# DavidRother/cooking_zoo

Measured on AMD Instinct MI355X. Metric: env-steps/sec at N parallel envs (1/2/4/8 GPU) + achieved HBM GB/s, higher is better.
Workload: dtype u8/u32 state, f64 obs+reward

## Files before the change

cooking_zoo_amd/csrc/cz_api.hip:

```cpp
#include <hip/hip_runtime.h>
#include <dlfcn.h>
#include <stdarg.h>
#include <stdio.h>
#include <stdlib.h>
#include <string.h>

#include <atomic>
#include <string>
#include <vector>

#include "../../include/cookingzoo.h"
#include "cz_launch.h"
#include "cz_generate.h"

using namespace cz;

constexpr int STAT_CHAINS = 256, STAT_COLS = 13;
__global__ __launch_bounds__(64) void k_stats_chains(const uint32_t *__restrict__ su, const double *__restrict__ sf,
                                                     const uint32_t *__restrict__ state, int RW, int N,
                                                     unsigned long long *__restrict__ part ) {
    const int chain = (int)blockIdx.x * 4 + ((int)threadIdx.x >> 4), col = (int)threadIdx.x & 15;
    const int widx = col == 0 ? (int)SU_STEPS : col == 1 ? (int)SU_EPISODES : col == 2 ? (int)SU_LENSUM : col == 3 ? (int)SU_TRUNC
                   : col == 4 ? (int)SU_TERM : col < 9 ? (int)SU_COMPLETED0 + col - 5 : 0;
    const int fidx = (col >= 9 && col < STAT_COLS) ? (int)SF_SUM0 + col - 9 : (int)SF_SUM0;
// ... 283 lines not shown
    void *comm = nullptr;
    int n_ranks = 1, rank = 0;
    int wt_override = -1;
    bool lean_enabled = true;
    bool lean_cfg_enabled = true;
    int last_step_variant = -1;
    int last_step_lean = -1;
    int last_step_mode = -1;
    bool huge = false;
    int instance = 0;
    unsigned long long *tl_base = nullptr;
    int32_t tl_cap = 0;
    int64_t tl_count = 0;
    bool graphs_enabled = true;
    bool ring_fused = false;
    int64_t n_ring_fused_steps = 0;
    int32_t graph_min_run = 48;
    int32_t ring_prefix = 0;
    int32_t ring_split = -1;
    bool few_queues = false;
    hipStream_t split_stream = nullptr;
    hipEvent_t ev_fork = nullptr, ev_join = nullptr;
    size_t zero_copy_bytes = (size_t)256 << 10;
    cz_stats *d_gather = nullptr;
    std::string err;
};

static thread_local std::string g_err;
static int ready(cz_handle h);
static int set_device(cz_handle h);
static int begin_ranged_call(cz_handle h, int64_t b, int64_t c);
static void mark_ranks(cz_handle h, int32_t first, int32_t count, int ok);
static int flush_updates(cz_handle h, bool force);

static int fail(cz_handle h, const char *fmt, ...) {
    char buf[512];
    va_list ap;
    va_start(ap, fmt);
    vsnprintf(buf, sizeof buf, fmt, ap);
    va_end(ap);
    if (h) h->err = buf; else g_err = buf;
    return 1;
}

#define HIPCHK(h, call)                                                                      \
    do {                                                                                     \
        hipError_t _e = (call);                                                              \
        if (_e != hipSuccess) return fail(h, "%s failed: %s", #call, hipGetErrorString(_e)); \
    } while (0)

extern "C" const char *cz_last_error(cz_handle h) { return h ? h->err.c_str() : g_err.c_str(); }

template <class T>
static int64_t read_counter(cz_handle h, const void *d_counter, const char *who) {
    T n = 0;
    if (hipSetDevice(h->cfg.device_id) != hipSuccess || hipStreamSynchronize(h->stream) != hipSuccess ||
        hipMemcpy(&n, d_counter, sizeof n, hipMemcpyDeviceToHost) != hipSuccess) { fail(h, "%s: copy failed", who); return -1; }
    return (int64_t)n;
}
static int pool_levels(cz_handle h, const uint8_t *level_of, int32_t n_levels, const char *misfit, std::vector<uint8_t> &levels) {
    levels.assign((size_t)h->n_layouts, 0);
    for (int i = 0; i < h->n_layouts; ++i) {
        const int lv = level_of ? level_of[i] : 0;
        if (lv >= n_levels) return fail(h, misfit, i, lv, n_levels);
        levels[(size_t)i] = (uint8_t)lv;
    }
// ... 310 lines not shown
    if (!h) return fail(nullptr, "null handle");
    HIPCHK(h, hipStreamSynchronize(h->stream));
    return 0;
}

static int encode_node(cz_handle h, int recipe, uint32_t j, uint32_t hw, uint32_t children, uint32_t *out) {
    const uint32_t cls = hw & 0xFF, cond = (hw >> 8) & 0xFF, counts = (hw >> 24) & 1;
    uint32_t w = children | (counts << 8);
    if (cls < 16) {
        w |= 0x200u | ((cls <= BLENDER ? cls : 7u) << 10);
    } else if (cls < 32) {
        const bool blender_food = (cls - 16) == CARROT || (cls - 16) == BANANA;
        uint32_t acc;
        if (cond & 0x10u) acc = cond & 0xFu;
        else if (cond == COND_NONE) acc = 0xFu;
        else if (cond == COND_CHOPPED) acc = 0xAu;
        else if (cond == COND_NOT_CHOPPED) acc = 0x5u;
        else if (cond == COND_MASHED) acc = blender_food ? 0xCu : 0u;
        else if (cond == COND_NOT_MASHED) acc = blender_food ? 0x3u : 0u;
        else return fail(h, "cz_load_recipes: recipe %d node %u: unknown condition code %u", recipe, j, cond);
        w |= 0x2000u | ((cls - 16) << 16) | (acc << 24);
    }
    *out = w;
    return 0;
}

extern "C" int cz_load_recipes(cz_handle h, const uint32_t *table, int32_t n, int32_t max_nodes) {
    if (!h || !table || n < 1 || n > 255 || (max_nodes != MAX_NODES && max_nodes != WIDE_NODES)) return fail(h, "cz_load_recipes: bad arguments");
    const bool wide = max_nodes == WIDE_NODES;
    const size_t row_words = wide ? 1 + 2 * WIDE_NODES : 1 + MAX_NODES;
    for (int i = 0; i < n; ++i)
        if (table[(size_t)i * row_words] > (uint32_t)max_nodes) return fail(h, "cz_load_recipes: recipe %d has more than %d nodes", i, max_nodes);
    HIPCHK(h, hipSetDevice(h->cfg.device_id));
    if (h->d_recipes) { HIPCHK(h, hipStreamSynchronize(h->stream)); HIPCHK(h, hipFree(h->d_recipes)); h->d_recipes = nullptr; h->P.recipes = nullptr; }
    size_t bytes = (size_t)n * row_words * 4;
    HIPCHK(h, hipMalloc(&h->d_recipes, bytes));
    std::vector<uint32_t> dev(table, table + (size_t)n * row_words);
    for (int i = 0; i < n; ++i) {
        uint32_t *row = dev.data() + (size_t)i * row_words;
        const uint32_t nn = row[0];
        for (uint32_t j = 0; j < (uint32_t)max_nodes; ++j) {
            if (wide) {
                if (j >= nn) { row[1 + 2 * j] = row[2 + 2 * j] = 0; continue; }
                if (encode_node(h, i, j, row[1 + 2 * j], 0, &row[1 + 2 * j])) return 1;
                row[2 + 2 * j] &= 0xFFFFu;
            } else {
                if (j >= nn) { row[1 + j] = 0; continue; }
                if (encode_node(h, i, j, row[1 + j], (row[1 + j] >> 16) & 0xFF, &row[1 + j])) return 1;
            }
        }
        row[0] = nn & 0xFFu;
    }
    HIPCHK(h, hipMemcpyAsync(h->d_recipes, dev.data(), bytes, hipMemcpyHostToDevice, h->stream));
    HIPCHK(h, hipStreamSynchronize(h->stream));
    h->n_recipes = n;
    h->P.recipes = h->d_recipes;
    h->tables_version++;
    h->n_partner = 0;
    h->n_goal_rows = 0;
    int sensitive = h->P.A > 2;
    for (int i = 0; i < n && !sensitive; ++i) {
        const uint32_t *row = table + (size_t)i * row_words;
        auto node = [&](uint32_t j) { return wide ? row[1 + 2 * j] : row[1 + j]; };
        auto kids = [&](uint32_t j) { return wide ? (row[2 + 2 * j] & 0xFFFFu) : ((row[1 + j] >> 16) & 0xFFu); };
        for (uint32_t j = 0; j < row[0] && !sensitive; ++j) {
            uint32_t cls = node(j) & 0xFF, children = kids(j);
            for (uint32_t c = 0; c < row[0]; ++c) {
                if (!((children >> c) & 1)) continue;
                uint32_t ccls = node(c) & 0xFF;
                bool pw = cls == FLOOR || cls == SWITCH || cls == BLOCK, cw = ccls == FLOOR || ccls == SWITCH || ccls == BLOCK;
                bool pd = cls >= 16 && cls < 32, cd = ccls >= 16 && ccls < 32;
                if ((pw && cd) || (pd && cw)) sensitive = 1;
            }
        }
    }
    h->P.walk_touches = sensitive;
    h->P.wide = wide ? 1 : 0;
    return 0;
}

static int validate_layouts(cz_handle h, const char *who, const uint32_t *init_records, const uint32_t *obs_desc, int32_t n) {
    for (size_t i = 0; i < (size_t)n * h->P.F; ++i) {
        uint32_t off = obs_desc[i] & 0xFFFFu, code4 = obs_desc[i] >> 16;
        uint32_t hw = off >> 1, code = code4 >> 2;
        bool ok = !(off & 1u) && !(code4 & 3u) && (code <= 2 || (code >= 4 && code < 4 + 2 * (uint32_t)h->P.A));
        const uint32_t cell0 = h->huge ? Img<16>::CELL0 : Img<1>::CELL0, ag0 = h->huge ? Img<16>::AG0 : Img<1>::AG0;
        const uint32_t zero = h->huge ? Img<16>::ZERO : Img<1>::ZERO;
        if (hw < cell0) ok = ok && (int)(hw / 6) < h->P.D;
        else if (hw < ag0) ok = ok && (int)((hw - cell0) / 4) < h->P.W * h->P.H;
        else if (hw < zero) ok = ok && (int)((hw - ag0) / 8) < h->P.A && ((hw - ag0) & 7u) < 7u;
        else ok = ok && hw == zero;
        if (!ok) return fail(h, "%s: bad observation descriptor %#x at %zu", who, obs_desc[i], i);
    }
    for (int32_t l = 0; l < n; ++l) {
        const uint32_t *r = init_records + (size_t)l * h->P.RW;
        for (int s2 = 0; s2 < h->P.D; ++s2)
            if (slot_dead_but_tagged(r[h->P.dyn0_off + s2], r[h->P.dyn1_off + s2]))
                return fail(h, "%s: layout %d: slot %d is not alive but carries a container tag", who, l, s2);
    }
    return 0;
}

extern "C" int cz_load_layouts(cz_handle h, const uint32_t *init_records, const uint32_t *obs_desc, int32_t n) {
    if (!h || !init_records || !obs_desc || n < 1 || n > 65535) return fail(h, "cz_load_layouts: bad arguments");
    if (validate_layouts(h, "cz_load_layouts", init_records, obs_desc, n)) return 1;
    HIPCHK(h, hipSetDevice(h->cfg.device_id));
    HIPCHK(h, hipStreamSynchronize(h->stream));
    if (h->copy_stream) HIPCHK(h, hipStreamSynchronize(h->copy_stream));
    if (h->n_layouts > 0 && n < h->n_layouts) {
        unsigned long long misfits = 0;
        HIPCHK(h, hipMemsetAsync(h->d_stats_part, 0, sizeof misfits, h->stream));
        hipLaunchKernelGGL(k_layout_misfits, dim3((unsigned)((h->P.N + 255) / 256)), dim3(256), 0, h->stream, h->d_state, h->P.RW, h->P.N,
                           (uint32_t)n, h->d_stats_part);
        HIPCHK(h, hipGetLastError());
        HIPCHK(h, hipMemcpyAsync(&misfits, h->d_stats_part, sizeof misfits, hipMemcpyDeviceToHost, h->stream));
        HIPCHK(h, hipStreamSynchronize(h->stream));
        if (misfits)
            return fail(h, "cz_load_layouts: %llu resident env record(s) refer to layouts >= %d of the pool being replaced (%d layouts); "
                           "cz_reset / cz_set_state them into the new range first, or load a pool that is not smaller",
                        misfits, n, h->n_layouts);
    }
    if (h->d_lay_block) { HIPCHK(h, hipFree(h->d_lay_block)); h->d_lay_block = nullptr; h->d_lay_init = nullptr; h->P.lay_init = nullptr; }
    if (h->d_lay_desc) { HIPCHK(h, hipFree(h->d_lay_desc)); h->d_lay_desc = nullptr; h->P.lay_desc = nullptr; }
    if (h->rank_stream) HIPCHK(h, hipStreamSynchronize(h->rank_stream));
    if (h->d_lay_rank) { HIPCHK(h, hipFree(h->d_lay_rank)); h->d_lay_rank = nullptr; }
    if (h->h_rank_stage) { HIPCHK(h, hipHostFree(h->h_rank_stage)); h->h_rank_stage = nullptr; }
    if (h->h_lay_stage) { HIPCHK(h, hipHostFree(h->h_lay_stage)); h->h_lay_stage = nullptr; }
    size_t b0 = (size_t)n * h->P.RW * 4, b1 = (size_t)n * h->P.F * 4;
    HIPCHK(h, hipMalloc(&h->d_lay_block, LAY_CTL_WORDS * 4 + b0));
    h->d_lay_init = h->d_lay_block + LAY_CTL_WORDS;
    HIPCHK(h, hipMalloc(&h->d_lay_desc, b1 + 16));
    HIPCHK(h, hipMemsetAsync(h->d_lay_block, 0, LAY_CTL_WORDS * 4, h->stream));
    HIPCHK(h, hipMemsetD32Async((hipDeviceptr_t)(h->d_lay_block + LC_GROUPS), 1, 1, h->stream));
    HIPCHK(h, hipMemsetAsync(h->d_lay_desc, 0, b1 + 16, h->stream));
    const size_t b2 = (size_t)n * h->P.W * h->P.H * sizeof(uint16_t);
    HIPCHK(h, hipMalloc(&h->d_lay_rank, b2));
    HIPCHK(h, hipMemsetAsync(h->d_lay_rank, 0, b2, h->stream));
    h->rank_ok.assign((size_t)n, 0);
    h->rank_missing = n;
    HIPCHK(h, hipMemcpyAsync(h->d_lay_init, init_records, b0, hipMemcpyHostToDevice, h->stream));
    HIPCHK(h, hipMemcpyAsync(h->d_lay_desc, obs_desc, b1, hipMemcpyHostToDevice, h->stream));
    HIPCHK(h, hipStreamSynchronize(h->stream));
    h->n_layouts = n;
    if (h->P.auto_reset & 2) h->spawn_layouts = -1;
    h->lay_groups = 1; h->lay_active = 0; h->upd_ranges.clear(); h->staged_on_copy.clear(); h->staged_on_main.clear(); h->copy_pending = false;
    h->tables_version++;
    h->P.lay_init = h->d_lay_init; h->P.lay_desc = h->d_lay_desc; h->P.L = n;
    return 0;
}

static int flush_updates(cz_handle h, bool force) {
    if (h->upd_ranges.empty()) return 0;
    const hipError_t q = hipEventQuery(h->ev_steps_issued);
    if (q != hipSuccess) (void)hipGetLastError();
    if (q != hipSuccess && !force) return 0;
    const hipStream_t st = q == hipSuccess ? h->copy_stream : h->stream;
    const size_t RWb = (size_t)h->P.RW * 4, Fb = (size_t)h->P.F * 4, L = (size_t)h->n_layouts;
    for (const auto &r : h->upd_ranges) {
        HIPCHK(h, hipMemcpyAsync(h->d_lay_init + (size_t)r.first * h->P.RW, h->h_lay_stage + (size_t)r.first * RWb, (size_t)r.count * RWb,
                                 hipMemcpyHostToDevice, st));
        HIPCHK(h, hipMemcpyAsync(h->d_lay_desc + (size_t)r.first * h->P.F, h->h_lay_stage + L * RWb + (size_t)r.first * Fb, (size_t)r.count * Fb,
                                 hipMemcpyHostToDevice, st));
    }
    if (st == h->copy_stream) {
        if (!h->staged_on_copy.empty() && hipEventQuery(h->ev_copy_done) == hipSuccess) h->staged_on_copy.clear();
        (void)hipGetLastError();
        HIPCHK(h, hipEventRecord(h->ev_copy_done, h->copy_stream));
        h->copy_pending = true;
        h->staged_on_copy.insert(h->staged_on_copy.end(), h->upd_ranges.begin(), h->upd_ranges.end());
    } else {
        if (!h->staged_on_main.empty() && hipEventQuery(h->ev_main_copy_done) == hipSuccess) h->staged_on_main.clear();
        (void)hipGetLastError();
        HIPCHK(h, hipEventRecord(h->ev_main_copy_done, h->stream));
        h->staged_on_main.insert(h->staged_on_main.end(), h->upd_ranges.begin(), h->upd_ranges.end());
    }
    h->upd_ranges.clear();
    return 0;
}

extern "C" int cz_update_layouts(cz_handle h, int32_t first, int32_t count, const uint32_t *init_records, const uint32_t *obs_desc) {
    if (ready(h)) return 1;
    if (first < 0 || count < 0 || first + count > h->n_layouts || (count > 0 && (!init_records || !obs_desc)))
        return fail(h, "cz_update_layouts: slots [%d, %d) outside the resident pool of %d layouts", first, first + count, h ? h->n_layouts : 0);
    if (count > 0 && validate_layouts(h, "cz_update_layouts", init_records, obs_desc, count)) return 1;
    if (set_device(h)) return 1;
    if (caller_capturing(h)) return fail(h, "cz_update_layouts: not inside a stream capture of the caller (it records an event on the captured stream)");
    const size_t RWb = (size_t)h->P.RW * 4, Fb = (size_t)h->P.F * 4, L = (size_t)h->n_layouts;
    if (!h->copy_stream) {
        HIPCHK(h, hipStreamCreateWithFlags(&h->copy_stream, hipStreamNonBlocking));
        HIPCHK(h, hipEventCreateWithFlags(&h->ev_copy_done, hipEventDisableTiming));
        HIPCHK(h, hipEventCreateWithFlags(&h->ev_steps_issued, hipEventDisableTiming));
        HIPCHK(h, hipEventCreateWithFlags(&h->ev_main_copy_done, hipEventDisableTiming));
    }
    if (!h->h_lay_stage) HIPCHK(h, hipHostMalloc((void **)&h->h_lay_stage, L * (RWb + Fb), hipHostMallocDefault));
    if (count == 0) return 0;
// ... 122 lines not shown
    G.img_ag0 = h->huge ? Img<16>::AG0 : Img<1>::AG0; G.img_zero = h->huge ? Img<16>::ZERO : Img<1>::ZERO;
    h->gen_layouts = h->n_layouts;
    return 0;
}

extern "C" int cz_generate_layouts(cz_handle h, int32_t first, int32_t count, uint64_t seed, uint32_t generation) {
    if (ready(h)) return 1;
    if (!h->d_gen_tables || h->gen_layouts != h->n_layouts)
        return fail(h, "cz_generate_layouts: level programs not loaded for this pool (cz_load_level_programs, again after cz_load_layouts)");
    if (first < 0 || count < 0 || (int64_t)first + count > h->n_layouts)
        return fail(h, "cz_generate_layouts: slots [%d, %d) outside the resident pool of %d layouts", first, first + count, h->n_layouts);
    if (count == 0) return 0;
    if (h->lay_groups > 1)
        for (int s = first; s < first + count; ++s) {
            const auto &sl = h->gen_slices[(size_t)s];
            const int part = sl.count / h->lay_groups;
            if (part > 0 && (s - sl.first) / part == h->lay_active)
                return fail(h, "cz_generate_layouts: slot %d is in part %d of its pool slice, which the envs draw from (cz_set_layout_group)", s, h->lay_active);
        }
    if (set_device(h)) return 1;
    if (caller_capturing(h)) {
        if (!h->upd_ranges.empty() || h->copy_pending)
            return fail(h, "cz_generate_layouts: a cz_update_layouts copy is outstanding, which a stream capture cannot be ordered behind");
    } else {
        if (flush_updates(h, true)) return 1;
        if (h->copy_pending) { HIPCHK(h, hipStreamWaitEvent(h->stream, h->ev_copy_done, 0)); h->copy_pending = false; }
    }
    if (h->P.RW > (CELL_WORD0 + 256 + 2 * 255 + 15) / 16 * 16) return fail(h, "cz_generate_layouts: record longer than the generator's staging");
    GenParams G = h->gen;
    G.lay_init = h->d_lay_init; G.lay_desc = h->d_lay_desc; G.lay_rank = h->d_lay_rank;
    G.seed = seed; G.generation = generation; G.first = first;
    hipLaunchKernelGGL(k_generate_layouts, dim3((unsigned)count), dim3(64), 0, h->stream, G);
    HIPCHK(h, hipGetLastError());
    h->n_layout_updates += count;
    mark_ranks(h, first, count, 1);
    return 0;
}
extern "C" int64_t cz_generate_failures(cz_handle h) {
    if (!h) return -1;
    if (!h->d_gen_tables) return 0;
    return read_counter<uint32_t>(h, h->d_gen_tables, "cz_generate_failures");
}

static int copy_back_and_wait(cz_handle h, hipError_t rc, void *dst, const void *src, size_t bytes) {
    if (rc == hipSuccess && dst) rc = hipMemcpyAsync(dst, src, bytes, hipMemcpyDeviceToHost, h->stream);
    const hipError_t rs = hipStreamSynchronize(h->stream);
    HIPCHK(h, rc);
    HIPCHK(h, rs);
    return 0;
}

static void mark_ranks(cz_handle h, int32_t first, int32_t count, int ok) {
    for (int32_t l = first; l < first + count; ++l) {
        h->rank_missing += (int)h->rank_ok[(size_t)l] - ok;
        h->rank_ok[(size_t)l] = (uint8_t)ok;
    }
}
static int check_range(cz_handle h, int64_t b, int64_t c) {
    if (!h) return fail(nullptr, "null handle");
    if (b < 0 || c < 0 || b + c > h->P.N) return fail(h, "env range [%lld, %lld) outside [0, %d)", (long long)b, (long long)(b + c), h->P.N);
    return 0;
}

extern "C" int cz_set_state(cz_handle h, int64_t b, int64_t c, const uint32_t *records) {
    if (check_range(h, b, c)) return 1;
    if (c == 0) return 0;
// ... 1249 lines not shown
```

cooking_zoo_amd/csrc/cz_device.h:

```cpp
#pragma once
#include <hip/hip_runtime.h>
#include <stdint.h>
#include <type_traits>

namespace cz {

constexpr int MAX_AGENTS = 4;
constexpr int MAX_NODES = 8;
constexpr int WIDE_NODES = 16;
constexpr int HDR_WORDS = 8;
constexpr int AGENT_WORD0 = HDR_WORDS;
constexpr int RET_WORD0 = HDR_WORDS + MAX_AGENTS;
constexpr int CELL_WORD0 = RET_WORD0 + 2 * MAX_AGENTS;

enum : uint32_t { FLOOR = 0, COUNTER, DELIVERSQUARE, SWITCH, BLOCK, CUTBOARD, BLENDER };
enum : uint32_t { PLATE = 0, ONION, TOMATO, LETTUCE, CARROT, CUCUMBER, BANANA, APPLE, WATERMELON, BREAD };
enum : uint32_t { CELL_TYPE = 7, CELL_READY = 8, CELL_TOGGLE = 16, CELL_ACTIVE = 32, CELL_WALK = 64 };
enum : uint32_t { D_ALIVE = 1u << 24, D_CHOPPED = 2u << 24, D_MASHED = 4u << 24, D_FREE = 8u << 24, D_DONE = 6u << 24 };
enum : uint32_t { COND_NONE = 0, COND_CHOPPED, COND_MASHED, COND_NOT_CHOPPED, COND_NOT_MASHED };
enum : uint32_t { W_T = 0, W_MARKS, W_LAYOUT, W_STATUS, W_EPISODE, W_RECIPES, W_POOL, W_MARKS_HI };
enum : uint32_t { ST_DONE = 1, ST_TERM = 2, ST_TRUNC = 4 };
constexpr int LUT_Y0 = 63, LUT_ZERO = 126, LUT_ONE = 127;
constexpr int LUT_NDONE0 = 128, LUT_CH0 = 132, LUT_MA0 = 136, LUT_CF0 = 140, LUT_OR0 = 144;
enum : uint32_t { SU_EPISODES = 0, SU_STEPS, SU_LENSUM, SU_TRUNC, SU_TERM, SU_COMPLETED0, SU_LAST_LENGTH = 9, SU_LAST_EPISODE, SU_LAST_FLAGS,
// ... 95 lines not shown
#define CZ_PRIO 1
#endif
#if CZ_PRIO
#define CZ_SETPRIO(p) __builtin_amdgcn_s_setprio(p)
#else
#define CZ_SETPRIO(p) do { } while (0)
#endif
__device__ __forceinline__ uint32_t rfl(uint32_t v) { return __builtin_amdgcn_readfirstlane(v); }
__device__ __forceinline__ uint32_t rdl(uint32_t v, int l) { return __builtin_amdgcn_readlane(v, l); }
__device__ __forceinline__ uint64_t ballot(bool p) { return __builtin_amdgcn_ballot_w64(p); }
__device__ __forceinline__ bool lanes(uint64_t m) { return __builtin_amdgcn_inverse_ballot_w64(m); }
extern "C" __device__ uint32_t __cz_writelane(uint32_t, uint32_t, uint32_t) __asm("llvm.amdgcn.writelane.i32");
__device__ __forceinline__ uint32_t wrl(uint32_t value, int lane, uint32_t into) { return __cz_writelane(value, (uint32_t)lane, into); }

__host__ __device__ inline uint32_t action_hash(uint64_t seed, int64_t env_global, int agent, uint32_t step, uint32_t n) {
    uint32_t x = (uint32_t)seed ^ ((uint32_t)(seed >> 32) * 0x9E3779B1u);
    x ^= (uint32_t)env_global * 0x85EBCA6Bu + (uint32_t)((uint64_t)env_global >> 32) * 0x27D4EB2Fu;
    x ^= ((uint32_t)agent + 1u) * 0xC2B2AE35u;
    x ^= (step + 1u) * 0x165667B1u;
    x ^= x >> 16; x *= 0x7FEB352Du; x ^= x >> 15; x *= 0x846CA68Bu; x ^= x >> 16;
    x += step * 0x9E3779B9u;
    x ^= x >> 16; x *= 0x7FEB352Du; x ^= x >> 15; x *= 0x846CA68Bu; x ^= x >> 16;
    return (uint32_t)(((uint64_t)x * (uint64_t)n) >> 32);
}
__host__ __device__ inline uint32_t next_layout(int64_t env_global, uint32_t episode, uint32_t pool_word, uint32_t n_layouts,
                                                uint32_t groups = 1u, uint32_t active = 0u) {
    uint32_t base = pool_word & 0xFFFFu, count = pool_word >> 16;
    if (count == 0) { base = 0; count = n_layouts; }
    if (groups > 1u) { count /= groups; base += active * count; }
    return base + (uint32_t)(((uint64_t)env_global + (uint64_t)episode * 7919u) % count);
}
constexpr int LAY_CTL_WORDS = 16;
enum : uint32_t { LC_GROUPS = 0, LC_ACTIVE = 1 };

struct SpawnCfg {
    uint64_t seed;
    double despawn_rate, respawn_rate;
    uint32_t grace_period;
    uint32_t stride;
    const uint8_t *areas;
    const uint8_t *level_of_layout;
    uint32_t *exhausted;
};
static_assert(sizeof(SpawnCfg) == 56, "layout of the block behind Params::lut");
constexpr uint32_t SPAWN_CFG_OFFSET = 256 * 8 + 64 * 4;
constexpr uint32_t COORD_TABLE_OFFSET = SPAWN_CFG_OFFSET + 56, ROWSEL_TABLE_OFFSET = COORD_TABLE_OFFSET + 1024 * 4;
constexpr uint32_t LUT_BLOCK_BYTES = ROWSEL_TABLE_OFFSET + 64 * 4;
constexpr int SPAWN_GONE0 = 8, SPAWN_GRACE0 = 12;
__host__ __device__ inline uint32_t spawn_grace_bits(uint32_t grace_period, int n_agents) { return grace_period <= 31u ? 5u : 20u / (uint32_t)n_agents; }
__host__ __device__ inline uint32_t spawn_max_grace(int n_agents) { const uint32_t b = 20u / (uint32_t)n_agents; return b > 5u ? (1u << b) - 1u : 31u; }
__host__ __device__ inline uint32_t spawn_initial_status(uint32_t packed_grace, int n_agents) {
    const uint32_t grace = packed_grace & 0xFFFFFFu, bits = packed_grace >> 24;
    uint32_t st = 0;
    for (int a = 0; a < n_agents; ++a) st |= grace << (SPAWN_GRACE0 + bits * a);
    return st;
}

enum : uint32_t { HDR_LAYOUT = 1u, HDR_RECIPE = 2u, HDR_POOL = 4u };
__host__ __device__ inline uint32_t record_header_faults(uint32_t layout, uint32_t recipes, uint32_t pool, uint32_t L, int R, uint32_t n_recipes) {
    uint32_t faults = layout < L ? 0u : HDR_LAYOUT;
    for (int k = 0; k < R; ++k)
        if (((recipes >> (8 * k)) & 0xFFu) >= n_recipes) faults |= HDR_RECIPE;
    const uint32_t base = pool & 0xFFFFu, count = pool >> 16;
    if (count && base + count > L) faults |= HDR_POOL;
    return faults;
}
// ... 813 lines not shown
```

cooking_zoo_amd/csrc/cz_kernels.h:

```cpp
#pragma once
#include "cz_device.h"
#include <type_traits>

namespace cz {

#ifdef CZ_PROFILE
#define CZ_STAMP(i)                                                                                    \
    do {                                                                                               \
        unsigned long long _t;                                                                         \
        __builtin_amdgcn_sched_barrier(0);                                                             \
        asm volatile("s_memrealtime %0\n\ts_waitcnt lgkmcnt(0)" : "=s"(_t)::"memory");                 \
        __builtin_amdgcn_sched_barrier(0);                                                             \
        if (lane == 0 && P.stamps) P.stamps[(size_t)env * 16 + (i)] = _t;                               \
    } while (0)
#elif defined(CZ_MARKERS)
#define CZ_STAMP(i) asm volatile("; CZ_MARK " #i)
#else
#define CZ_STAMP(i) do { } while (0)
#endif

typedef const __attribute__((address_space(4))) Params *KParams;
struct StepArgsMirror { uint32_t *a; const int32_t *b; const double *c; int32_t i[8]; Params p; };
struct LeanArgsMirror { uint32_t *a; const int32_t *b; const double *c; int32_t i[8]; LeanParams p; };
static_assert(offsetof(LeanArgsMirror, p) == LEADING_SCALAR_BYTES && offsetof(StepArgsMirror, p) == LEADING_SCALAR_BYTES, "leading scalars");
// ... 153 lines not shown

template <class PB>
__device__ __forceinline__ uint32_t load_row_selector(const PB &P, int lane) { return ldg<uint32_t>(P.lut, ROWSEL_TABLE_OFFSET + (uint32_t)lane * 4u); }
template <class PB>
__device__ __forceinline__ uint32_t load_recipe_rows(const PB &P, uint32_t recipes, uint32_t sel) {
    const uint32_t id = (recipes >> (sel & 0xFFu)) & 0xFFu;
    return ldg<uint32_t>(P.recipes, __umul24(id, (1u + MAX_NODES) * 4u) + (sel >> 8));
}
template <class PB>
__device__ __forceinline__ uint32_t load_recipe_rows(const PB &P, uint32_t recipes, int lane) {
    return load_recipe_rows(P, recipes, load_row_selector(P, lane));
}

template <int OPL, int CPL, int NA, bool LEAN = false, class PB>
__device__ __forceinline__ void all_marks(const PB &P, Env<OPL, CPL, NA> &e, const Ctx &cx, uint32_t rowv, Lds<CPL> &s) {
    uint32_t lo = 0, hi = 0;
    if (!LEAN && __builtin_expect(P.wide != 0, 0)) {
#pragma nounroll
        for (int r = 0; r < P.R; ++r) {
            const uint32_t id = (e.recipes >> (8 * r)) & 0xFFu;
            const uint32_t m = Ops<OPL, CPL, NA, 3>::recipe_marks_wide(e, cx, P.recipes + (size_t)id * (1 + 2 * WIDE_NODES), s.locs);
            if (r < 2) lo |= m << (16 * r); else hi |= m << (16 * (r - 2));
        }
    } else {
        if constexpr (CPL <= 4) {
            lo = Ops<OPL, CPL, NA, 3>::recipe_marks_cells(e, cx, rowv, 0xFu, P.R, s.locs);
        } else {
#pragma nounroll
            for (int r = 0; r < P.R; ++r) lo |= Ops<OPL, CPL, NA, 3>::recipe_marks(e, cx, rowv, 9 * r, s.locs) << (8 * r);
        }
    }
    e.marks = lo; e.marks_hi = hi;
}

template <class PB>
__device__ __forceinline__ uint32_t load_submask(const PB &P, int lane) { return ldg<uint32_t>(P.lut, (uint32_t)(LUT_SIZE * 8 + lane * 4)); }

__device__ __forceinline__ void init_lut(const Params &P, double *lut, int tid, int nthreads) {
    for (int i = tid; i < LUT_SIZE; i += nthreads) lut[i] = ldg<double>(P.lut, (uint32_t)i * 8u);
}

template <int CPL> struct CoordWords { uint32_t w[CPL]; };
template <int CPL, class PB>
__device__ __forceinline__ CoordWords<CPL> load_coord_words(const PB &P, int lane) {
    CoordWords<CPL> cw;
#pragma unroll
    for (int k = 0; k < CPL; ++k) cw.w[k] = ldg<uint32_t>(P.lut, COORD_TABLE_OFFSET + (uint32_t)(lane + 64 * k) * 4u);
    return cw;
}
template <int CPL>
__device__ __forceinline__ void init_lds(const Ctx &cx, Lds<CPL> &s, const CoordWords<CPL> &cw) {
    const int lane = cx.lane;
    s.img[Img<CPL>::ZERO] = (uint16_t)(LUT_ABSENT * 8);
    uint32_t *img32 = reinterpret_cast<uint32_t *>(s.img);
#pragma unroll
    for (int k = 0; k < CPL; ++k) {
        const uint32_t c = (uint32_t)(lane + 64 * k);
        img32[(Img<CPL>::CELL0 >> 1) + 2 * c] = cw.w[k];
    }
}
template <int CPL, class PB>
__device__ __forceinline__ void init_lds(const PB &P, const Ctx &cx, Lds<CPL> &s) {
    const int lane = cx.lane;
    s.img[Img<CPL>::ZERO] = (uint16_t)(LUT_ABSENT * 8);
    uint32_t *img32 = reinterpret_cast<uint32_t *>(s.img);
#pragma unroll
// ... 186 lines not shown
        else { CZ_OBS_WRITE_ROWS(0); }
#undef CZ_OBS_WRITE_ROWS
    }
    if (!LEAN && P.F > 128 * OBS_PAIRS) load_desc(P, e.layout, 0, cx.lane, dsc);
    __builtin_amdgcn_wave_barrier();
}

struct StepOut {
    double myrew;
    uint32_t term, trunc;
    bool stepped, finished;
    bool header;
    uint32_t gone;
#ifdef CZ_TIMELINE
    uint32_t dbg;
#endif
};

#define CZ_RARE(hint, x) ((hint) ? __builtin_expect(!!(x), 0) : !!(x))
template <int OPL, int CPL, int NA, int SCHEME, bool FUSED, bool LEAN, class PB>
__device__ __forceinline__ void step_env(const PB &P, unsigned kp_off, Env<OPL, CPL, NA> &e, const Ctx &cx, uint32_t acts,
                                         int64_t env_global, uint32_t &rowv, Lds<CPL> &lds, uint32_t (&dsc)[OBS_CHUNK], Dirty &dt, StepOut &o) {
    using O = Ops<OPL, CPL, NA, SCHEME>;
    o.myrew = 0.0;
    o.term = 0; o.trunc = 0; o.stepped = false; o.finished = false; o.header = false; o.gone = 0u;
#ifdef CZ_TIMELINE
    o.dbg = 0u;
#endif
    const bool spawning = !LEAN && (P.auto_reset & 2) != 0;
    const SpawnCfg *const spawn_cfg = reinterpret_cast<const SpawnCfg *>(reinterpret_cast<const char *>(P.lut) + SPAWN_CFG_OFFSET);
    if (CZ_RARE(FUSED, (e.status & ST_DONE) != 0u)) {
        o.header = true;
        if (P.auto_reset & 1) {
            e.episode += 1;
            const uint32_t *const lay0 = late_params<block_of<PB>>(kp_off)->lay_init;
            typedef const __attribute__((address_space(4))) uint32_t *kconst_u32;
            const kconst_u32 ctl = (kconst_u32)(lay0 - LAY_CTL_WORDS);
            uint32_t lay = next_layout(env_global, e.episode, e.pool, (uint32_t)P.L, ctl[LC_GROUPS], ctl[LC_ACTIVE]);
            uint32_t recipes = e.recipes, episode = e.episode, pool = e.pool;
            load_env<OPL, CPL, NA, LEAN>(P, e, cx, lay0 + (size_t)lay * P.RW);
            e.t = 0; e.layout = lay; e.status = 0; e.episode = episode; e.recipes = recipes; e.pool = pool;
            if (spawning) {
                typedef const __attribute__((address_space(4))) SpawnCfg *kcfg;
                e.status = spawn_initial_status(((kcfg)spawn_cfg)->grace_period, NA);
            }
            all_marks<OPL, CPL, NA, LEAN>(P, e, cx, rowv, lds);
            if (LEAN || P.obs) load_desc(P, lay, 0, cx.lane, dsc);
            dt.cells = 1; dt.touched = 1; dt.interacted = 1;
        } else {
            o.term = (e.status & ST_TERM) ? 1u : 0u;
            o.trunc = (e.status & ST_TRUNC) ? 1u : 0u;
        }
        return;
    }
    o.stepped = true;
    e.t += 1;
#if defined(CZ_PROFILE)
    const int lane = cx.lane; const long long env = env_global - P.env_id_base;
#endif
    O::perform_agent_actions(e, cx, acts, dt);
    CZ_STAMP(2);
    O::progress_and_link(e, cx, dt);
    if (spawning) {
        o.gone = O::handle_agent_spawn(e, cx, spawn_cfg, env_global);
        o.header = true;
    }
    CZ_STAMP(3);
    const bool truncated = (int)e.t >= P.max_steps;
    const uint32_t before = e.marks;
    uint32_t after = before;
    o.myrew = cx.lane < NA ? P.reward_idle : 0.0;
    if (dt.moved & (uint32_t)P.walk_touches) { dt.touched = 1; dt.kinds = ~0ull; }
    if (dt.kinds & 0xFull) dt.kinds = ~0ull;
    bool done = false;
    if (!LEAN && __builtin_expect(P.wide != 0, 0)) {
        if (dt.touched) {
            uint32_t lo = 0, hi = 0;
#pragma nounroll
            for (int r = 0; r < P.R; ++r) {
                const uint32_t id = (e.recipes >> (8 * r)) & 0xFFu;
// ... 398 lines not shown
```

cooking_zoo_amd/csrc/cz_launch.h:

```cpp
#pragma once
#include "cz_kernels.h"
#include "cz_offstep.h"
#include "cz_query.h"

namespace cz {

struct Launchers {
    hipError_t (*step)(const Params &, hipStream_t, StepChoice);
    hipError_t (*reset)(const Params &, hipStream_t, int64_t, int, const int32_t *, const uint32_t *, const uint32_t *, double *);
    hipError_t (*observe)(const Params &, hipStream_t, int64_t, int, double *, uint8_t *);
    bool has_lean;
    hipError_t (*observe_f32)(const Params &, hipStream_t, int64_t, int, float *);
    hipError_t (*reset_where)(const Params &, hipStream_t, const uint8_t *, const int32_t *, double *, float *, uint8_t *, unsigned long long *);
    hipError_t (*restore_where)(const Params &, hipStream_t, const int32_t *, const uint32_t *, int64_t, uint32_t, double *, float *, uint8_t *,
                                unsigned long long *);
    hipError_t (*set_tasks)(const Params &, hipStream_t, const uint8_t *, const uint32_t *, const uint32_t *, uint32_t, uint64_t, uint32_t,
                            unsigned long long *);
    hipError_t (*observe_grid)(const Params &, hipStream_t, int64_t, int, int32_t, uint32_t *, uint8_t *, float *, int32_t *);
    hipError_t (*navigate)(const Params &, hipStream_t, int64_t, int, int32_t, uint32_t, const int32_t *, int32_t *, int32_t *, uint16_t *);
    hipError_t (*partner)(const Params &, hipStream_t, int, const PartnerArgs &);
    hipError_t (*action_effects)(const Params &, hipStream_t, int, const EffectsArgs &);
    hipError_t (*render)(const Params &, hipStream_t, int, const RenderArgs &);
};

template <int OPL, int CPL, bool HAS_LEAN = false>
struct Inst {
    static hipError_t step(const Params &P, hipStream_t st, StepChoice c) {
        if constexpr (HAS_LEAN) {
            if (c.lean && c.cfg >= 0) {
                if (c.cfg != lean_cfg_of(P)) return hipErrorInvalidValue;
                const LeanParams B = lean_block_of(P);
                int row = 0;
#define CZ_X(a, s, r, ea, wt) if (c.cfg == row++) return launch_step_kernel<CPL>(k_step_lean_cfg<OPL, CPL, a, s, r, ea, wt>, P, B, st);
                CZ_LEAN_CFGS(CZ_X)
#undef CZ_X
                return hipErrorInvalidValue;
            }
        }
        return with_agents(P.A, [&](auto na) {
            return with_scheme(P.scheme, [&](auto scheme) {
                constexpr int NA = decltype(na)::value, S = decltype(scheme)::value;
                if (c.lean) {
                    if constexpr (HAS_LEAN) return launch_step_kernel<CPL>(k_step_lean<OPL, CPL, NA, S>, P, lean_block_of(P), st);
                    return hipErrorInvalidValue;
                }
                switch (c.mode) {
                case STEP: return launch_step_kernel<CPL>(k_step<OPL, CPL, NA, S, STEP>, P, st);
                case ROLLOUT: return launch_step_kernel<CPL>(k_step<OPL, CPL, NA, S, ROLLOUT>, P, st);
                case ROLLOUT_ACTIONS: return launch_step_kernel<CPL>(k_step<OPL, CPL, NA, S, ROLLOUT_ACTIONS>, P, st);
                case STEP_CODES: return launch_step_kernel<CPL>(k_step<OPL, CPL, NA, S, STEP_CODES>, P, st);
// ... 4 lines not shown
                case ROLLOUT_ACTIONS_F32: return launch_step_kernel<CPL>(k_step<OPL, CPL, NA, S, ROLLOUT_ACTIONS_F32>, P, st);
                }
                return hipErrorInvalidValue;
            });
        });
    }
#define CZ_LAUNCH_PER_ENV(K, envs, ...)                                                                                             \
    with_agents(P.A, [&](auto na) {                                                                                                 \
        hipLaunchKernelGGL((K<OPL, CPL, decltype(na)::value>), dim3((unsigned)(envs)), dim3(64), 0, st, P, __VA_ARGS__);            \
        return hipGetLastError();                                                                                                   \
    })
    static hipError_t reset(const Params &P, hipStream_t st, int64_t b, int n, const int32_t *lay, const uint32_t *rec,
                            const uint32_t *pool, double *obs) {
        return CZ_LAUNCH_PER_ENV(k_reset, n, b, lay, rec, pool, obs);
    }
    static hipError_t observe(const Params &P, hipStream_t st, int64_t b, int n, double *obs, uint8_t *codes) {
        return CZ_LAUNCH_PER_ENV(k_observe, n, b, obs, codes);
    }
    static hipError_t observe_f32(const Params &P, hipStream_t st, int64_t b, int n, float *obs) {
        return CZ_LAUNCH_PER_ENV(k_observe_f32, n, b, obs);
    }
    static hipError_t reset_where(const Params &P, hipStream_t st, const uint8_t *mask, const int32_t *lay, double *obs, float *obs32,
                                  uint8_t *codes, unsigned long long *refused) {
        return CZ_LAUNCH_PER_ENV(k_reset_where, P.N, mask, lay, obs, obs32, codes, refused);
    }
    static hipError_t restore_where(const Params &P, hipStream_t st, const int32_t *slot, const uint32_t *records, int64_t capacity,
                                    uint32_t n_recipes, double *obs, float *obs32, uint8_t *codes, unsigned long long *refused) {
        return CZ_LAUNCH_PER_ENV(k_restore_where, P.N, slot, records, capacity, n_recipes, obs, obs32, codes, refused);
    }
    static hipError_t set_tasks(const Params &P, hipStream_t st, const uint8_t *mask, const uint32_t *ids, const uint32_t *list, uint32_t K,
                                uint64_t seed, uint32_t n_recipes, unsigned long long *refused) {
        return CZ_LAUNCH_PER_ENV(k_set_tasks, P.N, mask, ids, list, K, seed, n_recipes, refused);
    }
    static hipError_t observe_grid(const Params &P, hipStream_t st, int64_t b, int n, int32_t extended, uint32_t *bits, uint8_t *grid8,
                                   float *grid32, int32_t *agent_xy) {
        return CZ_LAUNCH_PER_ENV(k_observe_grid, n, b, extended, bits, grid8, grid32, agent_xy);
    }
    static hipError_t navigate(const Params &P, hipStream_t st, int64_t b, int n, int32_t T, uint32_t flags, const int32_t *target,
                               int32_t *action, int32_t *steps, uint16_t *field) {
        return CZ_LAUNCH_PER_ENV(k_navigate, n, b, T, flags, target, action, steps, field);
    }
    static hipError_t partner(const Params &P, hipStream_t st, int n, const PartnerArgs &G) { return CZ_LAUNCH_PER_ENV(k_partner, n, G); }
    static hipError_t action_effects(const Params &P, hipStream_t st, int n, const EffectsArgs &G) {
        return with_agents(P.A, [&](auto na) {
            return with_scheme(P.scheme, [&](auto scheme) {
                constexpr int NA = decltype(na)::value, S = decltype(scheme)::value;
                hipLaunchKernelGGL((k_action_effects<OPL, CPL, NA, S>), dim3((unsigned)n * (unsigned)NA), dim3(64), 0, st, P, G);
                return hipGetLastError();
            });
        });
    }
    static hipError_t render(const Params &P, hipStream_t st, int n, const RenderArgs &G) {
        return with_agents(P.A, [&](auto na) {
            hipLaunchKernelGGL((k_render<OPL, CPL, decltype(na)::value>), dim3((unsigned)n * (unsigned)P.H, (G.P + RENDER_BAND - 1u) / RENDER_BAND), dim3(RENDER_THREADS), 0, st,
                               P, G);
            return hipGetLastError();
        });
    }
#undef CZ_LAUNCH_PER_ENV
    static Launchers launchers() {
        Launchers L{};
        L.step = &step; L.reset = &reset; L.observe = &observe; L.has_lean = HAS_LEAN; L.observe_f32 = &observe_f32;
        L.reset_where = &reset_where; L.restore_where = &restore_where; L.observe_grid = &observe_grid; L.navigate = &navigate;
        L.partner = &partner; L.action_effects = &action_effects; L.render = &render; L.set_tasks = &set_tasks;
        return L;
    }
};

Launchers launchers_small();
Launchers launchers_large();
Launchers launchers_huge();

}
```

cooking_zoo_amd/csrc/cz_offstep.h:

```cpp
#pragma once
#include "cz_kernels.h"

namespace cz {

__device__ __forceinline__ void init_lut_f32(const Params &P, float *lutf, int lane) {
    for (int i = lane; i < LUT_SIZE; i += 64) lutf[i] = (float)ldg<double>(P.lut, (uint32_t)i * 8u);
}
template <class T>
__device__ __forceinline__ T *row_of(T *base, size_t i, size_t pitch) { return base ? base + i * pitch : nullptr; }
template <int OPL, int CPL, int NA>
__device__ __forceinline__ void write_forms(const Params &P, const Env<OPL, CPL, NA> &e, const Ctx &cx, Lds<CPL> &lds, double *lut, float *lutf,
                                            double *obs, float *obs32, uint8_t *codes, size_t row) {
    const uint32_t submask = load_submask(P, cx.lane);
    if (obs || codes) {
        if (obs) init_lut(P, lut, cx.lane, 64);
        uint32_t dsc[OBS_CHUNK];
        load_desc(P, e.layout, 0, cx.lane, dsc);
        observe(P, e, cx, lds, lut, dsc, submask, row_of(obs, row, (size_t)NA * P.F), true, true, row_of(codes, row, (size_t)NA * codes_pitch(P.F)));
    }
    if (obs32) {
        init_lut_f32(P, lutf, cx.lane);
        if (!(obs || codes)) build_image<OPL, CPL, NA>(P, e, cx, lds, submask, true, true);
        write_rows_f32<OPL, CPL, NA>(P, e, cx, lds, lutf, obs32 + row * NA * P.F, nullptr);
    }
}
template <int OPL, int CPL, int NA>
__device__ __forceinline__ void begin_episode(const Params &P, Env<OPL, CPL, NA> &e, const Ctx &cx, Lds<CPL> &lds, uint32_t *rec, uint32_t lay,
                                              uint32_t episode, uint32_t recipes, uint32_t pool) {
    load_env(P, e, cx, P.lay_init + (size_t)lay * P.RW);
    e.t = 0; e.layout = lay; e.status = 0; e.episode = episode; e.recipes = recipes; e.pool = pool;
    if (P.auto_reset & 2)
        e.status = spawn_initial_status(rfl(reinterpret_cast<const SpawnCfg *>(reinterpret_cast<const char *>(P.lut) + SPAWN_CFG_OFFSET)->grace_period), NA);
    uint32_t rowv = load_recipe_rows(P, e.recipes, cx.lane);
    all_marks(P, e, cx, rowv, lds);
    store_env(P, e, cx, rec, true, true);
    if (cx.lane < MAX_AGENTS) reinterpret_cast<double *>(rec + RET_WORD0)[cx.lane] = 0.0;
}

template <int OPL, int CPL, int NA>
__global__ __launch_bounds__(64) void k_reset(const Params P, int64_t env_begin, const int32_t *__restrict__ layout_ids,
                                              const uint32_t *__restrict__ recipe_words, const uint32_t *__restrict__ pool_words,
                                              double *obs_out) {
    __shared__ Lds<CPL> lds;
    __shared__ double lut[LUT_SIZE];
    const int i = blockIdx.x;
    Ctx cx{P.W, P.H, P.D, P.W * P.H, (int)threadIdx.x};
    init_lds<CPL>(P, cx, lds);
    Env<OPL, CPL, NA> e;
    uint32_t *rec = P.state + (size_t)(env_begin + i) * P.RW;
    const uint32_t old_episode = rfl(rec[W_EPISODE]);
    begin_episode(P, e, cx, lds, rec, rfl((uint32_t)layout_ids[i]), old_episode, rfl(recipe_words[i]), rfl(pool_words[i]));
    write_forms(P, e, cx, lds, lut, nullptr, obs_out, nullptr, nullptr, (size_t)i);
}

template <int OPL, int CPL, int NA>
__global__ __launch_bounds__(64) void k_observe(const Params P, int64_t env_begin, double *obs_out, uint8_t *codes_out) {
    __shared__ Lds<CPL> lds;
    __shared__ double lut[LUT_SIZE];
    const int i = blockIdx.x;
    Ctx cx{P.W, P.H, P.D, P.W * P.H, (int)threadIdx.x};
    init_lds<CPL>(P, cx, lds);
    Env<OPL, CPL, NA> e;
    load_env(P, e, cx, P.state + (size_t)(env_begin + i) * P.RW);
    write_forms(P, e, cx, lds, lut, nullptr, obs_out, nullptr, codes_out, (size_t)i);
}

template <int OPL, int CPL, int NA>
__global__ __launch_bounds__(64) void k_observe_f32(const Params P, int64_t env_begin, float *obs_out) {
    __shared__ Lds<CPL> lds;
    __shared__ float lutf[LUT_SIZE];
    const int i = blockIdx.x;
    Ctx cx{P.W, P.H, P.D, P.W * P.H, (int)threadIdx.x};
    init_lds<CPL>(P, cx, lds);
    Env<OPL, CPL, NA> e;
    load_env(P, e, cx, P.state + (size_t)(env_begin + i) * P.RW);
    write_forms(P, e, cx, lds, nullptr, lutf, nullptr, obs_out, nullptr, (size_t)i);
}

template <int OPL, int CPL, int NA>
__global__ __launch_bounds__(64) void k_reset_where(const Params P, const uint8_t *__restrict__ mask, const int32_t *__restrict__ layout_ids,
                                                    double *obs_out, float *obs32_out, uint8_t *codes_out, unsigned long long *refused) {
    __shared__ Lds<CPL> lds;
    __shared__ double lut[LUT_SIZE];
    __shared__ float lutf[LUT_SIZE];
    const uint32_t env = blockIdx.x;
    const int lane = (int)threadIdx.x;
    uint32_t *rec = P.state + (size_t)env * P.RW;
    uint32_t old_status = 0u;
    if (mask) {
        if (rfl((uint32_t)mask[env]) == 0u) return;
        old_status = rfl(rec[W_STATUS]);
    } else {
        old_status = rfl(rec[W_STATUS]);
        if (!(old_status & ST_DONE)) return;
    }
    const int32_t want = layout_ids ? (int32_t)rfl((uint32_t)layout_ids[env]) : -1;
    if (want >= P.L) {
        if (lane == 0) atomicAdd(refused, 1ull);
        return;
    }
    const uint32_t old_t = rfl(rec[W_T]), episode = rfl(rec[W_EPISODE]) + 1u, recipes = rfl(rec[W_RECIPES]), pool = rfl(rec[W_POOL]);
    if (!(old_status & ST_DONE) && lane == 0) P.stat_u[(size_t)env * SU_WORDS + SU_STEPS] += old_t;
    uint32_t lay = (uint32_t)want;
    if (want < 0) {
        const uint32_t *ctl = P.lay_init - LAY_CTL_WORDS;
        lay = next_layout(P.env_id_base + (int64_t)env, episode, pool, (uint32_t)P.L, rfl(ctl[LC_GROUPS]), rfl(ctl[LC_ACTIVE]));
    }
    Ctx cx{P.W, P.H, P.D, P.W * P.H, lane};
    init_lds<CPL>(P, cx, lds);
    Env<OPL, CPL, NA> e;
    begin_episode(P, e, cx, lds, rec, lay, episode, recipes, pool);
    write_forms(P, e, cx, lds, lut, lutf, obs_out, obs32_out, codes_out, env);
}

template <int OPL, int CPL>
constexpr int record_chunks() { return ((CELL_WORD0 + 16 * CPL + 128 * OPL + 15) / 16 * 16 + 63) / 64; }
template <int OPL, int CPL, int NA>
__global__ __launch_bounds__(64) void k_restore_where(const Params P, const int32_t *__restrict__ slot, const uint32_t *__restrict__ records,
                                                      int64_t capacity, uint32_t n_recipes, double *obs_out, float *obs32_out,
                                                      uint8_t *codes_out, unsigned long long *refused) {
    __shared__ Lds<CPL> lds;
    __shared__ double lut[LUT_SIZE];
    __shared__ float lutf[LUT_SIZE];
    constexpr int NW = record_chunks<OPL, CPL>();
    const uint32_t env = blockIdx.x;
    const int lane = (int)threadIdx.x;
    int64_t s = (int64_t)env;
    if (slot) {
        const int32_t v = (int32_t)rfl((uint32_t)slot[env]);
        if (v < 0) return;
        s = v;
    }
    if (s >= capacity) {
        if (lane == 0) atomicAdd(refused, 1ull);
        return;
    }
    const uint32_t *row = records + (size_t)s * P.RW;
    uint32_t *rec = P.state + (size_t)env * P.RW;
    const uint32_t RW = (uint32_t)P.RW;
    uint32_t raw[NW];
#pragma unroll
    for (int k = 0; k < NW; ++k) raw[k] = ldg<uint32_t>(row, min((uint32_t)lane + 64u * k, RW - 1u) * 4u);
    Ctx cx{P.W, P.H, P.D, P.W * P.H, lane};
    Env<OPL, CPL, NA> e;
// ... 32 lines not shown
    const int lane = (int)threadIdx.x;
    uint32_t *rec = P.state + (size_t)env * P.RW;
    if (mask) {
        if (rfl((uint32_t)mask[env]) == 0u) return;
    } else {
        if (rfl(rec[W_T]) != 0u) return;
    }
    uint32_t want;
    if (ids) want = rfl(ids[env]);
    else want = rfl(list[task_draw(seed, P.env_id_base + (int64_t)env, rfl(rec[W_EPISODE]), K)]);
    bool bad = false;
    for (int r = 0; r < MAX_AGENTS; ++r) {
        if (r >= P.R) want |= 0xFFu << (8 * r);
        else if (((want >> (8 * r)) & 0xFFu) >= n_recipes) bad = true;
    }
    if (bad) {
        if (lane == 0) atomicAdd(refused, 1ull);
        return;
    }
    Ctx cx{P.W, P.H, P.D, P.W * P.H, lane};
    Env<OPL, CPL, NA> e;
    load_env(P, e, cx, rec);
    e.recipes = want;
    const uint32_t rowv = load_recipe_rows(P, e.recipes, lane);
    all_marks(P, e, cx, rowv, lds);
    uint32_t h = 0;
    h = wrl(e.marks, W_MARKS, h);
    h = wrl(e.recipes, W_RECIPES, h);
    h = wrl(e.marks_hi, W_MARKS_HI, h);
    const uint32_t ul = (uint32_t)lane;
    if (ul == W_MARKS || ul == W_RECIPES || (P.wide && ul == W_MARKS_HI)) stg<uint32_t>(rec, ul * 4u, h);
}

}
```

Before: 779.7 million.

## Precompute per-layout recipe marks table and use it on episode reset

Adds a per-layout table of initial recipe marks, indexed by layout and recipe id and stored after the layout init records. A new kernel fills it whenever layouts or recipes change. On auto-reset and begin_episode, the marks are then read with one small load per lane instead of rerunning all_marks over the recipe rows. This takes the recipe-evaluation work out of the hot reset path, at the cost of extra memory and upkeep every time layouts or recipes are updated.

```diff
diff --git a/cooking_zoo_amd/csrc/cz_api.hip b/cooking_zoo_amd/csrc/cz_api.hip
--- a/cooking_zoo_amd/csrc/cz_api.hip
+++ b/cooking_zoo_amd/csrc/cz_api.hip
@@ -339,6 +339,7 @@
 static int begin_ranged_call(cz_handle h, int64_t b, int64_t c);
 static void mark_ranks(cz_handle h, int32_t first, int32_t count, int ok);
 static int flush_updates(cz_handle h, bool force);
+static int refresh_layout_marks(cz_handle h, int32_t first, int32_t count, hipStream_t st);
 
 static int fail(cz_handle h, const char *fmt, ...) {
     char buf[512];
@@ -715,7 +716,11 @@
     for (int i = 0; i < n; ++i)
         if (table[(size_t)i * row_words] > (uint32_t)max_nodes) return fail(h, "cz_load_recipes: recipe %d has more than %d nodes", i, max_nodes);
     HIPCHK(h, hipSetDevice(h->cfg.device_id));
-    if (h->d_recipes) { HIPCHK(h, hipStreamSynchronize(h->stream)); HIPCHK(h, hipFree(h->d_recipes)); h->d_recipes = nullptr; h->P.recipes = nullptr; }
+    if (h->d_recipes) {
+        HIPCHK(h, hipStreamSynchronize(h->stream));
+        if (h->copy_stream) HIPCHK(h, hipStreamSynchronize(h->copy_stream));
+        HIPCHK(h, hipFree(h->d_recipes)); h->d_recipes = nullptr; h->P.recipes = nullptr;
+    }
     size_t bytes = (size_t)n * row_words * 4;
     HIPCHK(h, hipMalloc(&h->d_recipes, bytes));
     std::vector<uint32_t> dev(table, table + (size_t)n * row_words);
@@ -759,6 +764,17 @@
     }
     h->P.walk_touches = sensitive;
     h->P.wide = wide ? 1 : 0;
+    if (h->P.lay_init) {
+        if (h->copy_stream) HIPCHK(h, hipStreamSynchronize(h->copy_stream));
+        HIPCHK(h, hipMemsetAsync(const_cast<uint16_t *>(lay_marks_of(h->d_lay_init, h->n_layouts, h->P.RW)), 0, lay_marks_bytes(h->n_layouts), h->stream));
+        if (refresh_layout_marks(h, 0, h->n_layouts, h->stream)) return 1;
+    }
+    return 0;
+}
+
+static int refresh_layout_marks(cz_handle h, int32_t first, int32_t count, hipStream_t st) {
+    if (!h->P.recipes || !h->P.lay_init || count <= 0) return 0;
+    HIPCHK(h, h->kl.layout_marks(h->P, st, first, count, (uint32_t)h->n_recipes));
     return 0;
 }
 
@@ -810,11 +826,12 @@
     if (h->h_rank_stage) { HIPCHK(h, hipHostFree(h->h_rank_stage)); h->h_rank_stage = nullptr; }
     if (h->h_lay_stage) { HIPCHK(h, hipHostFree(h->h_lay_stage)); h->h_lay_stage = nullptr; }
     size_t b0 = (size_t)n * h->P.RW * 4, b1 = (size_t)n * h->P.F * 4;
-    HIPCHK(h, hipMalloc(&h->d_lay_block, LAY_CTL_WORDS * 4 + b0));
+    HIPCHK(h, hipMalloc(&h->d_lay_block, LAY_CTL_WORDS * 4 + b0 + lay_marks_bytes(n)));
     h->d_lay_init = h->d_lay_block + LAY_CTL_WORDS;
     HIPCHK(h, hipMalloc(&h->d_lay_desc, b1 + 16));
     HIPCHK(h, hipMemsetAsync(h->d_lay_block, 0, LAY_CTL_WORDS * 4, h->stream));
     HIPCHK(h, hipMemsetD32Async((hipDeviceptr_t)(h->d_lay_block + LC_GROUPS), 1, 1, h->stream));
+    HIPCHK(h, hipMemsetAsync(const_cast<uint16_t *>(lay_marks_of(h->d_lay_init, n, h->P.RW)), 0, lay_marks_bytes(n), h->stream));
     HIPCHK(h, hipMemsetAsync(h->d_lay_desc, 0, b1 + 16, h->stream));
     const size_t b2 = (size_t)n * h->P.W * h->P.H * sizeof(uint16_t);
     HIPCHK(h, hipMalloc(&h->d_lay_rank, b2));
@@ -829,7 +846,7 @@
     h->lay_groups = 1; h->lay_active = 0; h->upd_ranges.clear(); h->staged_on_copy.clear(); h->staged_on_main.clear(); h->copy_pending = false;
     h->tables_version++;
     h->P.lay_init = h->d_lay_init; h->P.lay_desc = h->d_lay_desc; h->P.L = n;
-    return 0;
+    return refresh_layout_marks(h, 0, n, h->stream);
 }
 
 static int flush_updates(cz_handle h, bool force) {
@@ -844,6 +861,7 @@
                                  hipMemcpyHostToDevice, st));
         HIPCHK(h, hipMemcpyAsync(h->d_lay_desc + (size_t)r.first * h->P.F, h->h_lay_stage + L * RWb + (size_t)r.first * Fb, (size_t)r.count * Fb,
                                  hipMemcpyHostToDevice, st));
+        if (refresh_layout_marks(h, r.first, r.count, st)) return 1;
     }
     if (st == h->copy_stream) {
         if (!h->staged_on_copy.empty() && hipEventQuery(h->ev_copy_done) == hipSuccess) h->staged_on_copy.clear();
@@ -1032,6 +1050,7 @@
     G.seed = seed; G.generation = generation; G.first = first;
     hipLaunchKernelGGL(k_generate_layouts, dim3((unsigned)count), dim3(64), 0, h->stream, G);
     HIPCHK(h, hipGetLastError());
+    if (refresh_layout_marks(h, first, count, h->stream)) return 1;
     h->n_layout_updates += count;
     mark_ranks(h, first, count, 1);
     return 0;
diff --git a/cooking_zoo_amd/csrc/cz_device.h b/cooking_zoo_amd/csrc/cz_device.h
--- a/cooking_zoo_amd/csrc/cz_device.h
+++ b/cooking_zoo_amd/csrc/cz_device.h
@@ -151,6 +151,11 @@
 }
 constexpr int LAY_CTL_WORDS = 16;
 enum : uint32_t { LC_GROUPS = 0, LC_ACTIVE = 1 };
+constexpr int LAY_MARK_IDS = 256;
+constexpr size_t lay_marks_bytes(int L) { return (size_t)L * LAY_MARK_IDS * sizeof(uint16_t); }
+__host__ __device__ inline const uint16_t *lay_marks_of(const uint32_t *lay_init, int L, int RW) {
+    return reinterpret_cast<const uint16_t *>(lay_init + (size_t)L * (size_t)RW);
+}
 
 struct SpawnCfg {
     uint64_t seed;
diff --git a/cooking_zoo_amd/csrc/cz_kernels.h b/cooking_zoo_amd/csrc/cz_kernels.h
--- a/cooking_zoo_amd/csrc/cz_kernels.h
+++ b/cooking_zoo_amd/csrc/cz_kernels.h
@@ -209,6 +209,25 @@
     }
     e.marks = lo; e.marks_hi = hi;
 }
+template <class PB>
+__device__ __forceinline__ uint32_t load_fresh_marks(const PB &P, const uint32_t *lay0, uint32_t lay, uint32_t recipes, int lane) {
+    const uint32_t id = (recipes >> (8u * ((uint32_t)lane & 3u))) & 0xFFu;
+    return ldg<uint16_t>(lay_marks_of(lay0, P.L, P.RW), (lay * (uint32_t)LAY_MARK_IDS + id) * 2u);
+}
+template <int OPL, int CPL, int NA, bool LEAN = false, class PB>
+__device__ __forceinline__ void fresh_marks(const PB &P, Env<OPL, CPL, NA> &e, uint32_t entries) {
+    const bool wide = !LEAN && P.wide != 0;
+    uint32_t lo = 0, hi = 0;
+#pragma unroll
+    for (int r = 0; r < MAX_AGENTS; ++r) {
+        if (r >= P.R) break;
+        const uint32_t m = rdl(entries, r);
+        if (!wide) lo |= m << (8 * r);
+        else if (r < 2) lo |= m << (16 * r);
+        else hi |= m << (16 * (r - 2));
+    }
+    e.marks = lo; e.marks_hi = hi;
+}
 
 template <class PB>
 __device__ __forceinline__ uint32_t load_submask(const PB &P, int lane) { return ldg<uint32_t>(P.lut, (uint32_t)(LUT_SIZE * 8 + lane * 4)); }
@@ -461,20 +480,24 @@
     if (CZ_RARE(FUSED, (e.status & ST_DONE) != 0u)) {
         o.header = true;
         if (P.auto_reset & 1) {
+#ifdef CZ_TIMELINE
+            o.dbg |= 16u;
+#endif
             e.episode += 1;
             const uint32_t *const lay0 = late_params<block_of<PB>>(kp_off)->lay_init;
             typedef const __attribute__((address_space(4))) uint32_t *kconst_u32;
             const kconst_u32 ctl = (kconst_u32)(lay0 - LAY_CTL_WORDS);
             uint32_t lay = next_layout(env_global, e.episode, e.pool, (uint32_t)P.L, ctl[LC_GROUPS], ctl[LC_ACTIVE]);
             uint32_t recipes = e.recipes, episode = e.episode, pool = e.pool;
+            const uint32_t fresh = load_fresh_marks(P, lay0, lay, recipes, cx.lane);
+            if (LEAN || P.obs) load_desc(P, lay, 0, cx.lane, dsc);
             load_env<OPL, CPL, NA, LEAN>(P, e, cx, lay0 + (size_t)lay * P.RW);
             e.t = 0; e.layout = lay; e.status = 0; e.episode = episode; e.recipes = recipes; e.pool = pool;
             if (spawning) {
                 typedef const __attribute__((address_space(4))) SpawnCfg *kcfg;
                 e.status = spawn_initial_status(((kcfg)spawn_cfg)->grace_period, NA);
             }
-            all_marks<OPL, CPL, NA, LEAN>(P, e, cx, rowv, lds);
-            if (LEAN || P.obs) load_desc(P, lay, 0, cx.lane, dsc);
+            fresh_marks<OPL, CPL, NA, LEAN>(P, e, fresh);
             dt.cells = 1; dt.touched = 1; dt.interacted = 1;
         } else {
             o.term = (e.status & ST_TERM) ? 1u : 0u;
diff --git a/cooking_zoo_amd/csrc/cz_launch.h b/cooking_zoo_amd/csrc/cz_launch.h
--- a/cooking_zoo_amd/csrc/cz_launch.h
+++ b/cooking_zoo_amd/csrc/cz_launch.h
@@ -16,6 +16,7 @@
                                 unsigned long long *);
     hipError_t (*set_tasks)(const Params &, hipStream_t, const uint8_t *, const uint32_t *, const uint32_t *, uint32_t, uint64_t, uint32_t,
                             unsigned long long *);
+    hipError_t (*layout_marks)(const Params &, hipStream_t, int32_t, int32_t, uint32_t);
     hipError_t (*observe_grid)(const Params &, hipStream_t, int64_t, int, int32_t, uint32_t *, uint8_t *, float *, int32_t *);
     hipError_t (*navigate)(const Params &, hipStream_t, int64_t, int, int32_t, uint32_t, const int32_t *, int32_t *, int32_t *, uint16_t *);
     hipError_t (*partner)(const Params &, hipStream_t, int, const PartnerArgs &);
@@ -86,6 +87,11 @@
                                 uint64_t seed, uint32_t n_recipes, unsigned long long *refused) {
         return CZ_LAUNCH_PER_ENV(k_set_tasks, P.N, mask, ids, list, K, seed, n_recipes, refused);
     }
+    static hipError_t layout_marks(const Params &P, hipStream_t st, int32_t first, int32_t count, uint32_t n_recipes) {
+        const uint32_t chunks = (n_recipes + (uint32_t)P.R - 1u) / (uint32_t)P.R;
+        hipLaunchKernelGGL((k_layout_marks<OPL, CPL>), dim3((unsigned)count * chunks), dim3(64), 0, st, P, (uint32_t)first, n_recipes, chunks);
+        return hipGetLastError();
+    }
     static hipError_t observe_grid(const Params &P, hipStream_t st, int64_t b, int n, int32_t extended, uint32_t *bits, uint8_t *grid8,
                                    float *grid32, int32_t *agent_xy) {
         return CZ_LAUNCH_PER_ENV(k_observe_grid, n, b, extended, bits, grid8, grid32, agent_xy);
@@ -116,7 +122,7 @@
         Launchers L{};
         L.step = &step; L.reset = &reset; L.observe = &observe; L.has_lean = HAS_LEAN; L.observe_f32 = &observe_f32;
         L.reset_where = &reset_where; L.restore_where = &restore_where; L.observe_grid = &observe_grid; L.navigate = &navigate;
-        L.partner = &partner; L.action_effects = &action_effects; L.render = &render; L.set_tasks = &set_tasks;
+        L.partner = &partner; L.action_effects = &action_effects; L.render = &render; L.set_tasks = &set_tasks; L.layout_marks = &layout_marks;
         return L;
     }
 };
diff --git a/cooking_zoo_amd/csrc/cz_offstep.h b/cooking_zoo_amd/csrc/cz_offstep.h
--- a/cooking_zoo_amd/csrc/cz_offstep.h
+++ b/cooking_zoo_amd/csrc/cz_offstep.h
@@ -25,14 +25,14 @@
     }
 }
 template <int OPL, int CPL, int NA>
-__device__ __forceinline__ void begin_episode(const Params &P, Env<OPL, CPL, NA> &e, const Ctx &cx, Lds<CPL> &lds, uint32_t *rec, uint32_t lay,
+__device__ __forceinline__ void begin_episode(const Params &P, Env<OPL, CPL, NA> &e, const Ctx &cx, uint32_t *rec, uint32_t lay,
                                               uint32_t episode, uint32_t recipes, uint32_t pool) {
+    const uint32_t fresh = load_fresh_marks(P, P.lay_init, lay, recipes, cx.lane);
     load_env(P, e, cx, P.lay_init + (size_t)lay * P.RW);
     e.t = 0; e.layout = lay; e.status = 0; e.episode = episode; e.recipes = recipes; e.pool = pool;
     if (P.auto_reset & 2)
         e.status = spawn_initial_status(rfl(reinterpret_cast<const SpawnCfg *>(reinterpret_cast<const char *>(P.lut) + SPAWN_CFG_OFFSET)->grace_period), NA);
-    uint32_t rowv = load_recipe_rows(P, e.recipes, cx.lane);
-    all_marks(P, e, cx, rowv, lds);
+    fresh_marks(P, e, fresh);
     store_env(P, e, cx, rec, true, true);
     if (cx.lane < MAX_AGENTS) reinterpret_cast<double *>(rec + RET_WORD0)[cx.lane] = 0.0;
 }
@@ -49,7 +49,7 @@
     Env<OPL, CPL, NA> e;
     uint32_t *rec = P.state + (size_t)(env_begin + i) * P.RW;
     const uint32_t old_episode = rfl(rec[W_EPISODE]);
-    begin_episode(P, e, cx, lds, rec, rfl((uint32_t)layout_ids[i]), old_episode, rfl(recipe_words[i]), rfl(pool_words[i]));
+    begin_episode(P, e, cx, rec, rfl((uint32_t)layout_ids[i]), old_episode, rfl(recipe_words[i]), rfl(pool_words[i]));
     write_forms(P, e, cx, lds, lut, nullptr, obs_out, nullptr, nullptr, (size_t)i);
 }
 
@@ -109,7 +109,7 @@
     Ctx cx{P.W, P.H, P.D, P.W * P.H, lane};
     init_lds<CPL>(P, cx, lds);
     Env<OPL, CPL, NA> e;
-    begin_episode(P, e, cx, lds, rec, lay, episode, recipes, pool);
+    begin_episode(P, e, cx, rec, lay, episode, recipes, pool);
     write_forms(P, e, cx, lds, lut, lutf, obs_out, obs32_out, codes_out, env);
 }
 
@@ -208,4 +208,22 @@
     if (ul == W_MARKS || ul == W_RECIPES || (P.wide && ul == W_MARKS_HI)) stg<uint32_t>(rec, ul * 4u, h);
 }
 
-}
+template <int OPL, int CPL>
+__global__ __launch_bounds__(64) void k_layout_marks(const Params P, uint32_t first, uint32_t n_recipes, uint32_t chunks) {
+    __shared__ Lds<CPL> lds;
+    const uint32_t lay = first + blockIdx.x / chunks, id0 = (blockIdx.x % chunks) * (uint32_t)P.R;
+    const int lane = (int)threadIdx.x;
+    Ctx cx{P.W, P.H, P.D, P.W * P.H, lane};
+    Env<OPL, CPL, MAX_AGENTS> e;
+    load_env(P, e, cx, P.lay_init + (size_t)lay * P.RW);
+    e.recipes = 0u;
+    for (int r = 0; r < MAX_AGENTS; ++r) e.recipes |= min(id0 + (uint32_t)r, n_recipes - 1u) << (8 * r);
+    const uint32_t rowv = load_recipe_rows(P, e.recipes, lane);
+    all_marks(P, e, cx, rowv, lds);
+    const uint32_t r = (uint32_t)lane & 3u;
+    const uint32_t m = P.wide ? ((r < 2u ? e.marks : e.marks_hi) >> (16u * (r & 1u))) & 0xFFFFu : (e.marks >> (8u * r)) & 0xFFu;
+    uint16_t *const table = const_cast<uint16_t *>(lay_marks_of(P.lay_init, P.L, P.RW));
+    if (lane < P.R && id0 + r < n_recipes) stg<uint16_t>(table, (lay * (uint32_t)LAY_MARK_IDS + id0 + r) * 2u, (uint16_t)m);
+}
+
+}
```

Result: no change. 786.6 million (median of 6 runs) (+0.9%).
